# encryptorion-lab/phantom-fhe

Measured on AMD Instinct MI355X. Metric: forward NTT limb-transforms/s at N=2^16, 45 RNS moduli, higher is better.
Workload: dtype u64; 1 GPU; CKKS N=2^16, 45 data limbs (+15 special), forward NTT of a batch of 16 ciphertext polynomials per step (720 limb-transforms, 360 MiB, HBM-resident; configs[2] parameter set); N=65536, limbs=45, special_limbs=15, parallelism=ciphertext-batch x1, launch=K steps enqueued by one library call (2 K eager kernel launches)

## Files before the change

### phantom-fhe_amd/csrc/pha_modup_conv.h

```cpp
#pragma once

namespace pha {

struct ConvLimbRec {
    u64 p, oninv;
    double fq, fqinv;
    uint32_t jo, prime, fpok, pad;
    u64 ratio1;
};
constexpr int kMcsMaxOut = 64;
__device__ __forceinline__ uint32_t uni32(uint32_t x) { return (uint32_t)__builtin_amdgcn_readfirstlane((int)x); }
__device__ __forceinline__ u64 uni64(u64 x) { return ((u64)uni32((uint32_t)(x >> 32)) << 32) | uni32((uint32_t)x); }

constexpr int kMcsWaves = 2;
constexpr int kMcsRegLimbs = 8;
constexpr int kRescRegLimbs = 15;
constexpr int kDownRegLimbs = 8;
constexpr int mcs_reg_limbs(int form) { return form == 1 ? kRescRegLimbs : form == 2 ? kDownRegLimbs : kMcsRegLimbs; }
constexpr int kMcsLogTile = 10;
template <class C, int ISZ_PAD, int FORM = 0>
__global__ __launch_bounds__(C::THREADS) __attribute__((amdgpu_waves_per_eu(kMcsWaves, kMcsWaves)))
void modup_conv_s1_kernel(const NttKArgs k, const ModupConvArgs m) {
    constexpr bool RESC = FORM == 1;
    static_assert(C::STRIDED && C::EPT == 4 && C::NR == 3 && C::r(0) == 2, "radix-4 strided pass, four coefficients per thread");
    constexpr int K = 4, LOGD = C::LOGT - 2;
    using Prog = PassProgram<C, true, EPI_NONE, false, 1, false>;
    extern __shared__ __attribute__((aligned(16))) unsigned char smem[];
    u64 *lds = reinterpret_cast<u64 *>(smem);
    uint2 *s_rows = reinterpret_cast<uint2 *>(smem + (size_t)C::LDS_WORDS * sizeof(u64));
    ConvLimbRec *s_rec = reinterpret_cast<ConvLimbRec *>(s_rows + m.max_osz * kBcRowPad);
    const int tid = threadIdx.x;
    const uint32_t z = blockIdx.z, tile = blockIdx.x;
    const uint32_t ci = z % m.beta, grp = z / m.beta;
    const BConvDev &d = m.convs[ci];
    const uint32_t n = 1u << k.log_n, isz = d.isz, osz = d.osz, pitch = d.row_pad;
    const bool r90 = uni32(d.r90) != 0;
    for (uint32_t e = tid; e < osz * kBcRowPad; e += C::THREADS) {
        const uint32_t j = e / kBcRowPad, i = e % kBcRowPad;
        s_rows[e] = i < pitch ? reinterpret_cast<const uint2 *>(d.mat30)[j * pitch + i] : uint2{0u, 0u};
    }
    for (uint32_t j = tid; j < osz; j += C::THREADS) {
        ConvLimbRec r;
        r.jo = j + (j >= d.pad_start ? d.pad_len : 0);
        r.prime = r.jo >= k.sel.remap_from ? r.jo + k.sel.remap_add : r.jo;
        r.p = k.mod[r.prime].value;
        r.oninv = d.oninv[j];
        r.fpok = 0; r.fq = 0.0; r.fqinv = 0.0; r.pad = 0;
        r.ratio1 = k.mod[r.prime].ratio1;
        if (k.fpinfo) {
            const FpInfo fi = k.fpinfo[r.prime];
            r.fpok = fi.ok; r.fq = fi.q; r.fqinv = fi.qinv;
        }
        s_rec[j] = r;
    }
    int v, hi, lo;
    decode_group<C, 0>(tid, v, hi, lo);
    uint32_t off[K];
#pragma unroll
    for (int kk = 0; kk < K; kk++) off[kk] = (uint32_t)(lo + (kk << LOGD)) * k.t2 + tile * C::V + (uint32_t)v;
    const u64 *src = m.src + (size_t)grp * m.src_group_stride + (size_t)d.src_limb * n;
    u64 *dig = k.out + (size_t)z * k.poly_stride;
    constexpr int RL = mcs_reg_limbs(FORM) < ISZ_PAD ? mcs_reg_limbs(FORM) : ISZ_PAD;
    uint2 *s_in = reinterpret_cast<uint2 *>(s_rec + m.max_osz);
    u32 ylo[RL][K], yhi[RL][K];
#pragma unroll
    for (int i = 0; i < ISZ_PAD; i++)
#pragma unroll
        for (int kk = 0; kk < K; kk++) {
            const u64 y = i < (int)isz ? src[(size_t)i * n + off[kk]] : 0;
            if (i < RL) {
                ylo[i][kk] = (u32)y & 0x3fffffffu;
                yhi[i][kk] = (u32)(y >> 30);
            } else {
                s_in[((i - RL) * K + kk) * C::THREADS + tid] = uint2{(u32)y & 0x3fffffffu, (u32)(y >> 30)};
            }
        }
    if (d.copy_own && m.own) {
        const u64 *own = m.own + (size_t)grp * m.own_group_stride + (size_t)d.src_limb * n;
        for (uint32_t i = 0; i < isz; i++)
#pragma unroll
            for (int kk = 0; kk < K; kk++) dig[(size_t)(d.src_limb + i) * n + off[kk]] = own[(size_t)i * n + off[kk]];
    }
    __syncthreads();
    auto convert4 = [&](uint32_t e, u64 p, u64 oninv, u64 *out) __attribute__((always_inline)) {
        const uint2 *row = s_rows + e * kBcRowPad;
        u64 ll[K], lh[K], hl[K], hh[K];
#pragma unroll
        for (int kk = 0; kk < K; kk++) ll[kk] = lh[kk] = hl[kk] = hh[kk] = 0;
#pragma unroll
// ... 141 lines not shown
```

### phantom-fhe_amd/csrc/pha_modup_ip.h

```cpp
#pragma once

namespace pha {

template <class C, int BETA, bool FP>
__device__ __forceinline__ void modup_ip_body(const NttKArgs &k, const ModupIpArgs &ip, uint32_t twr, uint32_t prime, uint32_t tile,
                                              u64 *lds, int tid) {
    constexpr int RL = C::NR - 1, r = C::r(RL), K = 1 << r, G = C::EPT >> r;
    static_assert(C::LOGT - C::s0(RL) - r == 0, "the last round holds runs of K consecutive coefficients");
    using Prog = PassProgram<C, true, EPI_NONE, false, 0, false>;
    const size_t n = (size_t)1 << k.log_n;
    const DModulus m = k.mod[prime];
    const u64 q = m.value;
    FpMod fm{};
    u64 accb[C::EPT], acca[C::EPT];
#pragma unroll
    for (int i = 0; i < C::EPT; i++) accb[i] = acca[i] = FP ? as_u64(0.0) : 0;
    size_t g0[G];
#pragma unroll
    for (int gi = 0; gi < G; gi++) {
        int v, hi, lo;
        decode_group<C, RL>(tid + C::THREADS * gi, v, hi, lo);
        g0[gi] = ((size_t)tile * C::V + v) * C::T + ((size_t)hi << r);
    }
#pragma unroll 1
    for (int b = 0; b < BETA; b++) {
        PassArgs a;
        full_tile_args<C, true, EPI_NONE, false>(k, twr, (uint32_t)b, tile, a);
        a.fp = FP;
        fm = a.fpm;
        u64 reg[C::EPT];
        if (ip.own && limb_excluded(k, twr, (uint32_t)b)) {
#pragma unroll
            for (int gi = 0; gi < G; gi++)
#pragma unroll
                for (int kk = 0; kk < K; kk += 2) {
                    const u64x2 w = *reinterpret_cast<const u64x2 *>(ip.own + (size_t)twr * n + g0[gi] + kk);
                    reg[gi * K + kk] = FP ? as_u64(fp_from_canon(w.x)) : w.x;
                    reg[gi * K + kk + 1] = FP ? as_u64(fp_from_canon(w.y)) : w.y;
                }
        } else {
            u64x2 twreg[C::TW_TOTAL];
            Prog::load_twiddles(a, tid, twreg);
            Prog::template run_pass<SEG_KEEP, true>(a, lds, tid, reg, twreg);
            if (!FP) {
#pragma unroll
                for (int i = 0; i < C::EPT; i++) reg[i] = csub(csub(csub(reg[i], q << 2), q << 1), q);
            }
        }
        const u64 *key = ip.evks[b];
#pragma unroll
        for (int gi = 0; gi < G; gi++)
#pragma unroll
            for (int kk = 0; kk < K; kk += 2) {
                const size_t id = (size_t)prime * n + g0[gi] + kk;
// ... 113 lines not shown
```

### phantom-fhe_amd/csrc/pha_ntt.hip

```cpp
#include "../../include/phantom_amd.h"
#include "pha_internal.h"
#include "pha_experiments.h"
#include "pha_ntt_core.h"

#include <atomic>
#include <type_traits>

namespace pha {

constexpr int kPassHoist = 0;
#ifndef PHA_NTT_PASS_ORDER
#define PHA_NTT_PASS_ORDER 1
#endif
#ifndef PHA_NTT_ORDER_INT_HEAD
#define PHA_NTT_ORDER_INT_HEAD 1
#endif
#if defined(PHA_EXPERIMENTS)
std::atomic<int> g_ntt_variant{kDefaultVariant};
static inline int ntt_variant() { return g_ntt_variant.load(std::memory_order_relaxed); }
std::atomic<int> g_whole14_min{1 << 30};
std::atomic<int> g_fused_split{0};
std::atomic<int> g_fused_lag{2};
std::atomic<int> g_fused_min_tiles{1 << 30};
extern std::atomic<int> g_bconv_split;
#else
static constexpr int ntt_variant() { return kDefaultVariant; }
#endif

struct NttKArgs {
    const u64 *in;
    u64 *out;
    u64 *mid;
    const u64x2 *tw;
    const DModulus *mod;
    const u64x2 *ninv;
    const u64x2 *w1ninv;
    const u64 *twf;
    const u64x2 *ninvf, *w1ninvf;
    const FpInfo *fpinfo;
    const u64 *scale;
    const u64 *scale_shoup;
    const u64 *aux;
    const u64 *aux2;
// ... 101 lines not shown
        if (EPI == EPI_FWD_KSRESCALE) a.aux2 += (size_t)z * k.aux2_stride;
    }
    if (EPI == EPI_INV_CANON_ADD) a.aux += (size_t)(z >> 1) * k.aux_pair_stride + (size_t)(z & 1) * k.aux_stride;
    if (muladd_epilogue(EPI)) {
        a.aux += (size_t)z * k.aux_stride;
        a.aux2 += (size_t)z * k.aux2_stride;
        if (a.aux3) a.aux3 += (size_t)z * k.aux3_stride;
    }
    if (FWD && (C::STRIDED || C::WHOLE) && k.pro_src) {
        const uint32_t prime = twr >= k.sel.remap_from ? twr + k.sel.remap_add : twr;
        a.in = k.pro_src + (size_t)z * k.pro_stride;
        a.pro_reduce = true;
        a.pro_ratio1 = k.mod[prime].ratio1;
        a.pro_half = bfv_lift_threshold(k.pro_t);
        a.pro_inc = bfv_lift_increment(a.q, k.pro_t);
        a.pro_k = k.pro_k;
        a.ratio0 = k.mod[prime].ratio0;
        a.ratio1 = a.pro_ratio1;
    }
}

template <class C, bool FWD, int EPI, bool FOLD, int HOIST, bool COH, int ONLY = 0, int PRO = PRO_NONE>
__device__ __forceinline__ void exec_pass(const PassArgs &a, u64 *lds, int tid) {
    u64 reg[C::EPT];
    u64x2 twreg[C::TW_TOTAL];
    using Prog = PassProgram<C, FWD, EPI, FOLD, HOIST, COH, PRO>;
    auto pass = [&](const PassArgs &pa) __attribute__((always_inline)) {
        Prog::load_twiddles(pa, tid, twreg);
        Prog::template run_pass<SEG_PLAIN, false>(pa, lds, tid, reg, twreg);
    };
    PHA_WITH_FP_KNOWN(a, ONLY != 2 && a.fp, pass);
}

template <class C, bool FWD, int EPI, bool FOLD>
__global__ __launch_bounds__(C::THREADS) void ntt_zloop_kernel(const NttKArgs k, const ZloopMap m) {
    static_assert(!C::WHOLE, "the batched form exists for the passes of the two-pass plans");
    extern __shared__ __attribute__((aligned(16))) unsigned char smem[];
    u64 *lds = reinterpret_cast<u64 *>(smem);
    __builtin_amdgcn_s_setprio(3);
    const int tid = threadIdx.x;
    uint32_t b = blockIdx.x;
    PassArgs a;
    if (b < m.int_blocks) {
        const uint32_t tile = b % m.tiles, rest = b / m.tiles, z = rest % k.batch, twr = k.sel.start + m.limb[rest / k.batch];
        if (limb_excluded(k, twr, z)) return;
        full_tile_args<C, FWD, EPI, FOLD>(k, twr, z, tile, a);
        exec_pass<C, FWD, EPI, FOLD, 0, false, 2>(a, lds, tid);
        return;
    }
    b -= m.int_blocks;
    const uint32_t tile = b % m.tiles, rest = b / m.tiles, zgroups = (k.batch + m.zper - 1) / m.zper;
    const uint32_t twr = k.sel.start + m.limb[m.n_int + rest / zgroups];
    const uint32_t z0 = (rest % zgroups) * m.zper, z1 = (z0 + m.zper < k.batch) ? z0 + m.zper : k.batch;
    full_tile_args<C, FWD, EPI, FOLD>(k, twr, z0, tile, a);
    using Prog = PassProgram<C, FWD, EPI, FOLD, 1, false>;
    a.fp = true;
    u64x2 twreg[C::TW_TOTAL];
    Prog::load_twiddles(a, tid, twreg);
    u64 regA[C::EPT], regB[C::EPT];
    auto args_of = [&](uint32_t z) __attribute__((always_inline)) {
        PassArgs b = a;
        const size_t dz = (size_t)(z - z0);
        b.in += dz * k.in_stride;
        b.out += dz * k.out_stride;
        if (EPI == EPI_FWD_MODDOWN || EPI == EPI_FWD_MODDOWN_ADD || EPI == EPI_FWD_KSRESCALE) b.aux += dz * k.aux_stride;
        if (EPI == EPI_FWD_KSRESCALE) b.aux2 += dz * k.aux2_stride;
        return b;
    };
    auto transform = [&](const PassArgs &b, u64 *reg) __attribute__((always_inline)) {
        Prog::template run_pass<SEG_PREFETCHED, true>(b, lds, tid, reg, twreg);
    };
    auto next = [&](uint32_t z) __attribute__((always_inline)) {
        while (z < z1 && limb_excluded(k, twr, z)) z++;
        return z;
    };
    uint32_t z = next(z0);
    if (z >= z1) return;
    Prog::prefetch(args_of(z), tid, regA);
    __builtin_amdgcn_s_setprio(0);
    for (;;) {
        uint32_t zn = next(z + 1);
        if (zn < z1) Prog::prefetch(args_of(zn), tid, regB);
        transform(args_of(z), regA);
        if (zn >= z1) break;
        z = zn;
        zn = next(z + 1);
        if (zn < z1) Prog::prefetch(args_of(zn), tid, regA);
        transform(args_of(z), regB);
        if (zn >= z1) break;
        z = zn;
    }
}

template <class C, bool FWD, int EPI, bool FOLD, int HOIST, int PRO = PRO_NONE>
__global__ __launch_bounds__(C::THREADS) void ntt_pass_kernel(const NttKArgs k, const PassOrder o) {
    extern __shared__ __attribute__((aligned(16))) unsigned char smem[];
    u64 *lds = reinterpret_cast<u64 *>(smem);

    __builtin_amdgcn_s_setprio(3);
    uint32_t tile = blockIdx.x, y = blockIdx.y, z = blockIdx.z;
    if (k.zfast_tiles) {
        const uint32_t b = blockIdx.x, per_chunk = k.zfast_run * k.batch, chunk = b / per_chunk, rem = b - chunk * per_chunk;
        z = rem / k.zfast_run;
        const uint32_t group = chunk * k.zfast_run + (rem - z * k.zfast_run);
        if (group >= k.zfast_tiles * k.sel.count) return;
        tile = group % k.zfast_tiles;
        y = group / k.zfast_tiles;
    }
#if PHA_NTT_PASS_ORDER
    else if (o.tiles) {
        if (!pass_order_decode(o, k.batch, blockIdx.x, blockIdx.y, blockIdx.z, y, z, tile)) return;
    }
#endif
    const uint32_t twr = k.sel.start + y;
    if (limb_excluded(k, twr, z)) return;
    PassArgs a;
    full_tile_args<C, FWD, EPI, FOLD>(k, twr, z, tile, a);
    exec_pass<C, FWD, EPI, FOLD, HOIST, false, 0, PRO>(a, lds, threadIdx.x);
}

static void raise_lds_limit(const void *kernel, size_t bytes, std::atomic<uint64_t> &raised) {
// ... 75 lines not shown
    if constexpr (FWD) {
        if (k.pro_small) {
            if constexpr (W::LOGT <= 13) {
                if (epi == EPI_FWD_MULADD) return launch_pass<W, true, EPI_FWD_MULADD, false, PRO_SMALL>(k, s);
                if (epi == EPI_FWD_NEG_MULADD) return launch_pass<W, true, EPI_FWD_NEG_MULADD, false, PRO_SMALL>(k, s);
                return launch_pass<W, true, EPI_FWD_CANON, false, PRO_SMALL>(k, s);
            } else {
                throw std::logic_error("ntt_forward: the sample lift has no one-workgroup form at this degree");
            }
        }
        dispatch_epi<true>(epi, [&](auto e) {
            if constexpr (e() == EPI_FWD_CANON) dispatch_pro(k, [&](auto p) { launch_pass<W, true, EPI_FWD_CANON, false, p()>(k, s); });
            else launch_pass<W, true, e(), false>(k, s);
        });
    } else {
        launch_inverse_last<W>(k, epi, s);
    }
}

template <class C>
static bool plan_zloop(const NttKArgs &k, ZloopMap &m) {
    if (k.pro_src || k.sel.count > 128) return false;
    uint8_t fp[128];
    for (uint32_t y = 0; y < k.sel.count; y++) {
        const uint32_t twr = k.sel.start + y, prime = twr >= k.sel.remap_from ? twr + k.sel.remap_add : twr;
        fp[y] = k.fpinfo != nullptr && (k.h_primes[prime] >> 50) == 0;
    }
    return zloop_plan(m, k.sel.count, fp, k.batch, (uint32_t)(((size_t)1 << k.log_n) >> C::LOGTILE), C::THREADS / 64, kZloopMinBatch);
}
template <class C, bool FWD, int EPI, bool FOLD>
static void launch_zloop(const NttKArgs &k, const ZloopMap &m, hipStream_t s) {
    NttKArgs kk = k;
    kk.zfast_tiles = 0;
    const size_t lds_bytes = (size_t)C::LDS_WORDS * sizeof(u64);
    hipLaunchKernelGGL((ntt_zloop_kernel<C, FWD, EPI, FOLD>), dim3(zloop_blocks(m, k.batch)), dim3(C::THREADS), lds_bytes, s, kk, m);
    check_launch();
}
template <class C>
static void launch_zloop_forward(const NttKArgs &k, const ZloopMap &m, int epi, hipStream_t s) {
    dispatch_epi<true>(epi, [&](auto e) { launch_zloop<C, true, e(), false>(k, m, s); });
}

constexpr size_t kLastLevelCacheBytes = (size_t)256 << 20;
static NttKArgs limb_range(const NttKArgs &k, uint32_t lo, uint32_t cnt) {
    NttKArgs h = k;
    h.sel.start = k.sel.start + lo;
    h.sel.count = cnt;
    return h;
}
static uint32_t order_parts(const NttKArgs &k) {
    const size_t bytes = ((size_t)k.sel.count * k.batch << k.log_n) * sizeof(u64);
    return PHA_NTT_PASS_ORDER == 2 && k.sel.count >= 2 && bytes > kLastLevelCacheBytes ? 2u : 1u;
}

template <class F>
static void for_each_order_part(const NttKArgs &k, const ZloopMap &m, int strided_logtile, F &&pair) {
    if (PHA_NTT_PASS_ORDER == 0) return pair(0u, k.sel.count, m, (const PassOrder *)nullptr);
    const uint32_t parts = order_parts(k), cut = pass_order_half(k.sel.count);
    for (uint32_t h = 0; h < parts; h++) {
        const uint32_t lo = h * cut, hi = parts == 1 ? k.sel.count : h ? k.sel.count : cut;
        const ZloopMap mh = parts == 1 ? m : zloop_sub(m, lo, hi, k.batch);
        const PassOrder o = pass_order_reverse(mh, (uint32_t)(((size_t)1 << k.log_n) >> strided_logtile), PHA_NTT_ORDER_INT_HEAD != 0);
        pair(lo, hi - lo, mh, &o);
    }
}

constexpr int kIpPlan = 3;
// ... 480 lines not shown
```

### phantom-fhe_amd/csrc/pha_ntt_core.h

```cpp
#pragma once
#include "pha_arith.h"
#include "pha_bfv_lift.h"
#include "pha_ckks_fft.h"
#include "pha_encrypt.h"

namespace pha {

constexpr int kTileElems = 4096;

enum Epilogue {
    EPI_NONE = 0,
    EPI_FWD_CANON = 1,
    EPI_FWD_MODDOWN = 2,
    EPI_INV_CANON = 3,
    EPI_INV_SCALE = 4,
    EPI_FWD_MODDOWN_ADD = 5,
    EPI_FWD_KSRESCALE = 6,
    EPI_INV_CANON_ADD = 7,
    EPI_FWD_MULADD = 8,
    EPI_FWD_NEG_MULADD = 9,
};
constexpr bool muladd_epilogue(int epi) { return epi == EPI_FWD_MULADD || epi == EPI_FWD_NEG_MULADD; }

enum Prologue {
    PRO_NONE = 0,
    PRO_LIFT = 1,
    PRO_CKKS = 2,
    PRO_SMALL = 3,
};

template <int LOGT_, bool STRIDED_, int R0_, int R1_, int R2_ = 0, int EPT_ = 16, bool OT_ = false, int LOGTILE_ = 12,
          bool WHOLE_ = false, int R3_ = 0>
struct PassCfg {
    static constexpr int EPT = EPT_;
    static constexpr bool OT = OT_ && !STRIDED_;
    static constexpr int LOGTILE = LOGTILE_;
    static constexpr int TILE = 1 << LOGTILE_;
    static constexpr int THREADS = TILE / EPT_;
    static_assert(LOGTILE_ >= LOGT_ && LOGTILE_ <= 14, "a tile holds whole transforms and fits the LDS budget (2^14 words + padding = 144 KiB of the 160 KiB)");
    static constexpr bool WAVE_LOCAL = TILE / EPT_ == 64;
    static constexpr bool WHOLE = WHOLE_ && !STRIDED_;
    static_assert((1 << R0_) <= EPT_ && (1 << R1_) <= EPT_ && (1 << R2_) <= EPT_ && (1 << R3_) <= EPT_, "radix exceeds registers");
    static_assert(!R3_ || R2_, "rounds are filled in order");
    static constexpr int LOGT = LOGT_;
    static constexpr int T = 1 << LOGT_;
    static constexpr int LOGV = LOGTILE_ - LOGT_;
    static constexpr int V = 1 << LOGV;
    static constexpr bool STRIDED = STRIDED_;
    static constexpr int NR = R3_ ? 4 : R2_ ? 3 : 2;
    static_assert(R0_ + R1_ + R2_ + R3_ == LOGT_, "round schedule must cover all stages");
    static_assert(LOGT_ >= 4 && LOGT_ <= 14, "tile transform length out of range");
    static_assert(THREADS >= 64, "a workgroup is at least one wavefront");
    static constexpr int r(int i) { return i == 0 ? R0_ : i == 1 ? R1_ : i == 2 ? R2_ : R3_; }
    static constexpr bool ot_round(int i) { return OT && i == NR - 1; }
    static constexpr int tw_count(int i) {
        return !r(i) ? 0 : ot_round(i) ? ((1 << r(i)) - 1) + (EPT_ >> r(i)) * r(i) : (EPT_ >> r(i)) * ((1 << r(i)) - 1);
    }
    static constexpr int tw_off(int i) {
        return i == 0 ? 0 : i == 1 ? tw_count(0) : i == 2 ? tw_count(0) + tw_count(1) : tw_count(0) + tw_count(1) + tw_count(2);
    }
    static constexpr int TW_TOTAL = tw_count(0) + tw_count(1) + tw_count(2) + tw_count(3);
    static constexpr int s0(int i) { return i == 0 ? 0 : i == 1 ? R0_ : i == 2 ? R0_ + R1_ : R0_ + R1_ + R2_; }
    static constexpr int PITCH = T + ((T >> 4) << 1);
    static constexpr int LDS_WORDS = STRIDED_ ? (T * V + (T >> 4) * 16) : (V * PITCH);
    static constexpr int lds_index(int e, int v) {
        return STRIDED_ ? (e * V + v + ((e >> 4) << 4)) : (v * PITCH + e + ((e >> 4) << 1));
    }
};

struct PassArgs {
    const u64 *in;
    u64 *out;
    const u64x2 *tw;
    const u64 *twd;
    u64 q;
    u32 tile;
    u32 rho0;
    u32 stride;
    u64x2 ninv, w1ninv;
    u64x2 scale;
    const u64 *aux;
    u64x2 scale2;
    const u64 *aux2;
    bool fp;
    FpMod fpm;
    bool pro_reduce;
    u64 pro_ratio1;
    u64 pro_half, pro_inc;
    u64 pro_k;
    u64 ratio0, ratio1;
    const u64 *aux3;
};

template <class C>
PHA_HD size_t global_index(const PassArgs &a, int e, int v) {
    if (C::STRIDED) return (size_t)e * a.stride + (size_t)a.tile * C::V + v;
    return ((size_t)a.tile * C::V + v) * C::T + e;
}

template <class C, int RI>
PHA_HD void decode_group(int g, int &v, int &hi, int &lo) {
// ... 256 lines not shown
        return u64x2{t.x, t.y};
    }
#endif
    return *p;
}
template <bool NT>
PHA_HD void gstore(u64 *p, u64 v) {
#if defined(__HIP_DEVICE_COMPILE__)
    if (NT) {
        __builtin_nontemporal_store(v, p);
        return;
    }
#endif
    *p = v;
}
template <bool NT>
PHA_HD void gstore2(u64x2 *p, u64x2 v) {
#if defined(__HIP_DEVICE_COMPILE__)
    if (NT) {
        __builtin_nontemporal_store(u64v2{v.x, v.y}, reinterpret_cast<u64v2 *>(p));
        return;
    }
#endif
    *p = v;
}

template <class C, int RI, bool FROM_GLOBAL, bool COH = false>
PHA_HD void round_load(const PassArgs &a, const u64 *lds, int tid, u64 *reg) {
    constexpr int r = C::r(RI), K = 1 << r, G = C::EPT >> r, s0 = C::s0(RI);
    constexpr int LOGD = C::LOGT - s0 - r;
#pragma unroll
    for (int gi = 0; gi < G; gi++) {
        int v, hi, lo;
        decode_group<C, RI>(tid + C::THREADS * gi, v, hi, lo);
        u64 *rg = reg + gi * K;
        const int e0 = (hi << (LOGD + r)) + lo;
        if (FROM_GLOBAL && COH) {
#if defined(__HIP_DEVICE_COMPILE__)
            if constexpr (!C::STRIDED && K == 8 && G == 1 && LOGD >= 1 && LOGD <= 6) {
                const bool odd = lo & 1;
                const u64 *base = a.in + global_index<C>(a, e0 - (odd ? 1 : 0) + ((odd ? 4 : 0) << LOGD), v);
                u64x2 w0, w1, w2, w3;
                asm volatile("global_load_dwordx4 %0, %4, off sc1\n\t"
                             "global_load_dwordx4 %1, %4, off offset:%5 sc1\n\t"
                             "global_load_dwordx4 %2, %4, off offset:%6 sc1\n\t"
                             "global_load_dwordx4 %3, %4, off offset:%7 sc1\n\t"
                             "s_waitcnt vmcnt(0)"
                             : "=&v"(w0), "=&v"(w1), "=&v"(w2), "=&v"(w3)
                             : "v"(base), "n"(8 << LOGD), "n"(16 << LOGD), "n"(24 << LOGD)
                             : "memory");
                const u64x2 w[4] = {w0, w1, w2, w3};
#pragma unroll
                for (int j = 0; j < 4; j++) {
                    const u64 send = odd ? w[j].x : w[j].y;
                    const u32 slo = (u32)__builtin_amdgcn_update_dpp(0, (int)(u32)send, 0xB1, 0xF, 0xF, false);
                    const u32 shi = (u32)__builtin_amdgcn_update_dpp(0, (int)(u32)(send >> 32), 0xB1, 0xF, 0xF, false);
                    const u64 recv = ((u64)shi << 32) | slo;
                    rg[j] = odd ? recv : w[j].x;
                    rg[4 + j] = odd ? w[j].y : recv;
                }
                continue;
            }
#endif
#pragma unroll
            for (int k = 0; k < K; k++) rg[k] = coherent_load(a.in + global_index<C>(a, e0 + (k << LOGD), v));
        } else if (FROM_GLOBAL) {
            if (!C::STRIDED && LOGD == 0) {
                const u64x2 *p = reinterpret_cast<const u64x2 *>(a.in + global_index<C>(a, e0, v));
#pragma unroll
                for (int k = 0; k < K; k += 2) {
                    u64x2 t = gload2<false>(p + (k >> 1));
                    rg[k] = t.x;
                    rg[k + 1] = t.y;
                }
            } else {
#pragma unroll
                for (int k = 0; k < K; k++) rg[k] = gload<false>(a.in + global_index<C>(a, e0 + (k << LOGD), v));
            }
        } else {
#pragma unroll
            for (int k = 0; k < K; k++) rg[k] = lds[C::lds_index(e0 + (k << LOGD), v)];
        }
    }
}

template <class C, int RI>
PHA_HD void round_load_tw(const PassArgs &a, int tid, u64x2 *twreg) {
    constexpr int r = C::r(RI), K = 1 << r, G = C::EPT >> r, s0 = C::s0(RI);
    if (C::ot_round(RI)) {
        static_assert(!C::ot_round(RI) || (C::THREADS % (1 << s0)) == 0, "groups of a thread must share hi");
        u64x2 *base = twreg + C::tw_off(RI);
        int v, hi, lo;
        decode_group<C, RI>(tid, v, hi, lo);
        load_group_twiddles<r>(base, a, (u32)hi);
#pragma unroll
        for (int gi = 0; gi < G; gi++) {
            decode_group<C, RI>(tid + C::THREADS * gi, v, hi, lo);
            const u32 rho = a.rho0 + a.tile * C::V + (u32)v;
#pragma unroll
            for (int j = 0; j < r; j++) base[(K - 1) + gi * r + j] = tw_entry(a, rho << (s0 + j));
        }
        return;
    }
#pragma unroll
    for (int gi = 0; gi < G; gi++) {
        int v, hi, lo;
        decode_group<C, RI>(tid + C::THREADS * gi, v, hi, lo);
        const u32 rho = C::STRIDED ? 1u : (a.rho0 + a.tile * C::V + (u32)v);
        const u32 base0 = (rho << s0) + (u32)hi;
        load_group_twiddles<r>(twreg + C::tw_off(RI) + gi * (K - 1), a, base0);
    }
}

template <class C, int RI, bool FWD, bool FOLD, bool RECENTRE = false, bool GSFULL = false>
PHA_HD void round_compute(const PassArgs &a, int tid, u64 *reg, const u64x2 *twreg) {
    constexpr int r = C::r(RI), K = 1 << r, G = C::EPT >> r;
    const u64 q4 = a.q << 2, nq = 0 - a.q;
    if (C::ot_round(RI)) {
        const u64x2 *tc = twreg + C::tw_off(RI);
#pragma unroll
        for (int gi = 0; gi < G; gi++) {
            u64 *rg = reg + gi * K;
            const u64x2 *tr = tc + (K - 1) + gi * r;
            if (a.fp) {
                if (FWD ? a.fpm.ct_light : a.fpm.gs_light) ot_round_fp<r, FWD, true>(rg, tc, tr, a.fpm);
                else ot_round_fp<r, FWD, false>(rg, tc, tr, a.fpm);
            } else {
                ot_round_int<r, FWD>(rg, tc, tr, q4, nq);
            }
        }
        return;
    }
    if (a.fp) {
#pragma unroll
        for (int gi = 0; gi < G; gi++) {
            u64 *rg = reg + gi * K;
            const u64x2 *t = twreg + C::tw_off(RI) + gi * (K - 1);
            if (FWD) {
                fp_ct_round<r>(rg, t, a.fpm);
                if (RECENTRE && !a.fpm.ct_light) {
// ... 7 lines not shown
                if (light) fp_gs_round<r, FOLD, true>(rg, t, a.fpm, a.ninv, a.w1ninv);
                else fp_gs_round<r, FOLD, false, stage0, canon_in>(rg, t, a.fpm, a.ninv, a.w1ninv);
            } else {
                if (GSFULL) {
                    constexpr bool canon = RI == C::NR - 1 && (!C::STRIDED || C::WHOLE);
                    fp_gs_round<r, FOLD, false, 0, canon>(rg, t, a.fpm, a.ninv, a.w1ninv);
                } else {
                    fp_gs_round<r, FOLD, true>(rg, t, a.fpm, a.ninv, a.w1ninv);
                }
                if (RECENTRE) {
#pragma unroll
                    for (int k = 0; k < K; k++) rg[k] = as_u64(fp_reduce(as_f64(rg[k]), a.fpm));
                }
            }
        }
        return;
    }
#pragma unroll
    for (int gi = 0; gi < G; gi++) {
        u64 *rg = reg + gi * K;
        const u64x2 *t = twreg + C::tw_off(RI) + gi * (K - 1);
        if (FWD) ct_round<r>(rg, t, q4, nq);
        else gs_round<r, FOLD>(rg, t, q4, nq, a.ninv, a.w1ninv);
    }
}

template <class C, int RI, bool TO_GLOBAL, int EPI>
PHA_HD void round_out(const PassArgs &a, u64 *lds, int tid, const u64 *reg) {
    constexpr int r = C::r(RI), K = 1 << r, G = C::EPT >> r, s0 = C::s0(RI);
    constexpr int LOGD = C::LOGT - s0 - r;
#pragma unroll
    for (int gi = 0; gi < G; gi++) {
        int v, hi, lo;
        decode_group<C, RI>(tid + C::THREADS * gi, v, hi, lo);
        const u64 *rg = reg + gi * K;
        const int e0 = (hi << (LOGD + r)) + lo;
        if (TO_GLOBAL) {
            if (!C::STRIDED && LOGD == 0) {
                const size_t g0 = global_index<C>(a, e0, v);
                u64x2 *p = reinterpret_cast<u64x2 *>(a.out + g0);
#pragma unroll
                for (int k = 0; k < K; k += 2) {
                    if constexpr (muladd_epilogue(EPI)) {
                        const bool has_p = EPI == EPI_FWD_NEG_MULADD && a.aux3 != nullptr;
                        const u64x2 f0 = reinterpret_cast<const u64x2 *>(a.aux + g0)[k >> 1], f1 = reinterpret_cast<const u64x2 *>(a.aux2 + g0)[k >> 1];
                        const u64x2 pl = has_p ? reinterpret_cast<const u64x2 *>(a.aux3 + g0)[k >> 1] : u64x2{0, 0};
                        u64x2 t;
                        t.x = apply_epilogue_muladd<EPI>(rg[k], a, f0.x, f1.x, pl.x);
                        t.y = apply_epilogue_muladd<EPI>(rg[k + 1], a, f0.y, f1.y, pl.y);
                        gstore2<false>(p + (k >> 1), t);
                        continue;
                    }
                    u64x2 aux{0, 0}, acc{0, 0};
                    if (EPI == EPI_FWD_MODDOWN || EPI == EPI_FWD_MODDOWN_ADD || EPI == EPI_FWD_KSRESCALE || EPI == EPI_INV_CANON_ADD)
                        aux = reinterpret_cast<const u64x2 *>(a.aux + g0)[k >> 1];
                    if (EPI == EPI_FWD_MODDOWN_ADD) acc = p[k >> 1];
                    if (EPI == EPI_FWD_KSRESCALE) acc = reinterpret_cast<const u64x2 *>(a.aux2 + g0)[k >> 1];
                    u64x2 t;
                    t.x = apply_epilogue_v<EPI>(rg[k], a, aux.x, acc.x);
                    t.y = apply_epilogue_v<EPI>(rg[k + 1], a, aux.y, acc.y);
                    gstore2<false>(p + (k >> 1), t);
                }
            } else {
#pragma unroll
                for (int k = 0; k < K; k++) {
                    const size_t gidx = global_index<C>(a, e0 + (k << LOGD), v);
                    gstore<false>(a.out + gidx, apply_epilogue<EPI>(rg[k], a, gidx));
                }
            }
        } else {
#pragma unroll
            for (int k = 0; k < K; k++) lds[C::lds_index(e0 + (k << LOGD), v)] = rg[k];
        }
    }
}

template <class C>
PHA_HD void tile_sync() {
#if defined(__HIP_DEVICE_COMPILE__)
    if constexpr (C::WAVE_LOCAL) {
        __builtin_amdgcn_fence(__ATOMIC_RELEASE, "wavefront");
        __builtin_amdgcn_wave_barrier();
        __builtin_amdgcn_fence(__ATOMIC_ACQUIRE, "wavefront");
    } else {
        __syncthreads();
    }
#endif
}

enum SegMode { SEG_PLAIN = 0, SEG_PREFETCHED = 1, SEG_KEEP = 2 };

template <class C, bool FWD, int EPI, bool FOLD, int HOIST = 1, bool COH = false, int PRO = PRO_NONE>
struct PassProgram {
    static constexpr int NSEG = C::NR;
    static constexpr int THREADS = C::THREADS;
    static constexpr bool FIRST_PASS = C::WHOLE || (FWD ? C::STRIDED : !C::STRIDED);
    static constexpr bool LAST_PASS = C::WHOLE || !(FWD ? C::STRIDED : !C::STRIDED);

    static constexpr double kFpLimit = 7.5;
    struct FpSched {
        bool recentre[4];
        bool full[4];
        double after[4];
    };
    static constexpr double fp_grow(double m, int stages, bool full) {
        if (!FWD) {
            if (full) return 2.0;
            for (int i = 0; i < stages; i++) m = 2.0 * m + 1e-6;
            return m;
        }
        for (int i = 0; i < stages; i++) m = full ? m + 0.5 + 1e-6 : 1.375 * m + 0.5 + 1e-6;
        return m;
    }
// ... 24 lines not shown
            if (C::ot_round(ri) && (sc.full[seg] || (FWD && sc.recentre[seg]))) return false;
        }
        return true;
    }
    static_assert(fp_sched_ok(), "FP64 path: a round would take the registers past 7.5 q (exactness needs < 8 q at 50 bits), or the schedule asks an on-the-fly-twiddle round to re-centre");

    PHA_HD static void fp_after_global_load(const PassArgs &a, u64 *reg) {
        if (!a.fp) return;
        if (!FIRST_PASS && !(FWD ? a.fpm.ct_light : a.fpm.gs_light)) return;
#pragma unroll
        for (int i = 0; i < C::EPT; i++)
            reg[i] = as_u64(FIRST_PASS ? fp_from_canon(reg[i]) : fp_reduce(as_f64(reg[i]), a.fpm));
    }
    PHA_HD static void fp_before_global_store(const PassArgs &a, u64 *reg) {
        if (!a.fp || !LAST_PASS) return;
        if (fp_epilogue(EPI)) return;
#pragma unroll
        for (int i = 0; i < C::EPT; i++) reg[i] = fp_to_canon(as_f64(reg[i]), a.fpm);
    }

    static constexpr int round_of(int seg) { return FWD ? seg : C::NR - 1 - seg; }
    PHA_HD static void load_twiddles(const PassArgs &a, int tid, u64x2 *twreg) {
        if (HOIST == 1) {
            round_load_tw<C, 0>(a, tid, twreg);
            round_load_tw<C, 1>(a, tid, twreg);
            if (C::NR >= 3) round_load_tw<C, 2>(a, tid, twreg);
            if (C::NR == 4) round_load_tw<C, 3>(a, tid, twreg);
        } else if (HOIST == 2) {
            round_load_tw<C, round_of(0)>(a, tid, twreg);
        }
    }
    template <int SEG>
    PHA_HD static void segment_twiddles(const PassArgs &a, int tid, u64x2 *twreg) {
        if (HOIST == 0) round_load_tw<C, round_of(SEG)>(a, tid, twreg);
        if (HOIST == 2 && SEG + 1 < C::NR) round_load_tw<C, round_of(SEG + 1 < C::NR ? SEG + 1 : SEG)>(a, tid, twreg);
    }

    template <int SEG, int MODE>
    PHA_HD static void segment(const PassArgs &a, u64 *lds, int tid, u64 *reg, u64x2 *twreg) {
        constexpr int RI = round_of(SEG);
        constexpr bool first = SEG == 0, last = SEG == C::NR - 1;
        static_assert(MODE != SEG_KEEP || (last && !first), "the kept segment is the last one of a multi-round pass");
        static_assert(MODE != SEG_KEEP || !(fp_sched().recentre[SEG] || fp_sched().full[SEG]), "a kept segment hands over what the rounds left");
        segment_twiddles<SEG>(a, tid, twreg);
        if constexpr (!(first && MODE == SEG_PREFETCHED)) round_load<C, RI, first, COH>(a, lds, tid, reg);
        if constexpr (first && MODE == SEG_PLAIN) {
#if defined(__HIP_DEVICE_COMPILE__)
            __builtin_amdgcn_s_setprio(0);
#endif
            if constexpr (PRO == PRO_LIFT) {
                static_assert(FWD && FIRST_PASS, "the plain lift is the load prologue of a forward transform's first pass");
#pragma unroll
                for (int i = 0; i < C::EPT; i++) reg[i] = bfv_lift_word(reg[i], a.pro_half, a.pro_inc);
            } else if constexpr (PRO == PRO_CKKS) {
                static_assert(FWD && FIRST_PASS, "round-and-reduce is the load prologue of a forward transform's first pass");
#pragma unroll
                for (int i = 0; i < C::EPT; i++) reg[i] = ckks_round_reduce64(as_f64(reg[i]), a.q, a.pro_ratio1);
            } else if constexpr (PRO == PRO_SMALL) {
                static_assert(FWD && FIRST_PASS, "the sample lift is the load prologue of a forward transform's first pass");
                if (a.pro_k) {
                    const DModulus dm{a.q, a.ratio0, a.ratio1};
                    const u64 kq = barrett64(a.pro_k, a.q, a.ratio1);
#pragma unroll
                    for (int i = 0; i < C::EPT; i++) reg[i] = small_lift_scaled(reg[i], kq, dm);
                } else {
#pragma unroll
                    for (int i = 0; i < C::EPT; i++) reg[i] = small_lift(reg[i], a.q);
                }
            } else if (FWD && FIRST_PASS && a.pro_reduce) {
#pragma unroll
                for (int i = 0; i < C::EPT; i++) reg[i] = barrett64(reg[i], a.q, a.pro_ratio1);
            }
        }
        static_assert(PRO == PRO_NONE || MODE == SEG_PLAIN, "the load prologue belongs to the pass that loads");
        if (first) fp_after_global_load(a, reg);
        if (FWD && C::WHOLE && C::LOGT >= 14 && SEG == 2 && a.fp) {
#pragma unroll
            for (int i = 0; i < C::EPT; i++) reg[i] = as_u64(fp_reduce(as_f64(reg[i]), a.fpm));
        }
        round_compute<C, RI, FWD, FOLD && RI == 0, fp_sched().recentre[SEG], fp_sched().full[SEG]>(a, tid, reg, twreg);
        if constexpr (MODE != SEG_KEEP) {
            if (last) fp_before_global_store(a, reg);
            round_out<C, RI, last, last ? EPI : (int)EPI_NONE>(a, lds, tid, reg);
        }
    }
    template <int SEG>
    PHA_HD static void run(const PassArgs &a, u64 *lds, int tid, u64 *reg, u64x2 *twreg) { segment<SEG, SEG_PLAIN>(a, lds, tid, reg, twreg); }
    template <int SEG>
    PHA_HD static void run_prefetched(const PassArgs &a, u64 *lds, int tid, u64 *reg, u64x2 *twreg) { segment<SEG, SEG_PREFETCHED>(a, lds, tid, reg, twreg); }
    template <int SEG>
    PHA_HD static void run_keep(const PassArgs &a, u64 *lds, int tid, u64 *reg, u64x2 *twreg) { segment<SEG, SEG_KEEP>(a, lds, tid, reg, twreg); }

    PHA_HD static void prefetch(const PassArgs &a, int tid, u64 *reg) { round_load<C, round_of(0), true>(a, nullptr, tid, reg); }

    template <int MODE, bool TAIL_SYNC, int SEG = 0>
    PHA_HD static void run_pass(const PassArgs &a, u64 *lds, int tid, u64 *reg, u64x2 *twreg) {
        constexpr bool last = SEG == NSEG - 1;
        segment<SEG, (MODE == SEG_KEEP && !last) ? (int)SEG_PLAIN : MODE>(a, lds, tid, reg, twreg);
        if constexpr (!last) {
            tile_sync<C>();
            run_pass<MODE, TAIL_SYNC, SEG + 1>(a, lds, tid, reg, twreg);
        } else if constexpr (TAIL_SYNC) {
            tile_sync<C>();
        }
    }
};

#define PHA_WITH_FP_KNOWN(a, cond, body) \
    if (cond) {                          \
        PassArgs b_ = (a);               \
        b_.fp = true;                    \
        body(b_);                        \
    } else {                             \
        PassArgs b_ = (a);               \
        b_.fp = false;                   \
        body(b_);                        \
    }

template <int LOGN, int VARIANT> struct NttPlan;
template <> struct NttPlan<12, 0> { using P1 = PassCfg<6, true, 3, 3>;  using P2 = PassCfg<6, false, 3, 3>; };
template <> struct NttPlan<13, 0> { using P1 = PassCfg<6, true, 3, 3>;  using P2 = PassCfg<7, false, 4, 3>; };
template <> struct NttPlan<14, 0> { using P1 = PassCfg<7, true, 4, 3>;  using P2 = PassCfg<7, false, 4, 3>; };
template <> struct NttPlan<15, 0> { using P1 = PassCfg<7, true, 4, 3>;  using P2 = PassCfg<8, false, 4, 4>; };
template <> struct NttPlan<16, 0> { using P1 = PassCfg<8, true, 4, 4>;  using P2 = PassCfg<8, false, 4, 4>; };
template <> struct NttPlan<17, 0> { using P1 = PassCfg<8, true, 4, 4>;  using P2 = PassCfg<9, false, 3, 3, 3>; };
template <> struct NttPlan<12, 1> { using P1 = PassCfg<6, true, 3, 3, 0, 8>;  using P2 = PassCfg<6, false, 3, 3, 0, 8>; };
template <> struct NttPlan<13, 1> { using P1 = PassCfg<6, true, 3, 3, 0, 8>;  using P2 = PassCfg<7, false, 3, 2, 2, 8>; };
template <> struct NttPlan<14, 1> { using P1 = PassCfg<7, true, 3, 2, 2, 8>;  using P2 = PassCfg<7, false, 3, 2, 2, 8>; };
template <> struct NttPlan<15, 1> { using P1 = PassCfg<7, true, 3, 2, 2, 8>;  using P2 = PassCfg<8, false, 3, 3, 2, 8>; };
template <> struct NttPlan<16, 1> { using P1 = PassCfg<8, true, 3, 3, 2, 8>;  using P2 = PassCfg<8, false, 3, 3, 2, 8>; };
template <> struct NttPlan<17, 1> { using P1 = PassCfg<8, true, 3, 3, 2, 8>;  using P2 = PassCfg<9, false, 3, 3, 3, 8>; };
template <> struct NttPlan<12, 2> { using P1 = PassCfg<6, true, 3, 3, 0, 8>;  using P2 = PassCfg<6, false, 3, 3, 0, 8, true>; };
template <> struct NttPlan<13, 2> { using P1 = PassCfg<6, true, 3, 3, 0, 8>;  using P2 = PassCfg<7, false, 3, 2, 2, 8, true>; };
// ... 169 lines not shown
```

Measured before the change: 2.657 million NTT/s.

## Use wave-local barriers for wave-owned NTT rounds and double-buffer zloop LDS

Remaps thread-to-group assignment so that, in non-strided multi-wave tiles, each wavefront owns contiguous blocks of groups. Later rounds whose data stays inside one wavefront can then synchronise with a wavefront barrier instead of the workgroup barrier. The batched zloop kernel alternates between two LDS areas so the trailing tail barrier can be dropped. A new hoist mode (3) loads the next round's twiddles after compute but is not enabled by default. The doubled LDS footprint could limit occupancy, and a static_assert caps it.

```diff
diff --git a/phantom-fhe_amd/csrc/pha_modup_conv.h b/phantom-fhe_amd/csrc/pha_modup_conv.h
--- a/phantom-fhe_amd/csrc/pha_modup_conv.h
+++ b/phantom-fhe_amd/csrc/pha_modup_conv.h
@@ -54,7 +54,7 @@
         s_rec[j] = r;
     }
     int v, hi, lo;
-    decode_group<C, 0>(tid, v, hi, lo);
+    decode_group<C, 0>(thread_group<C>(tid, 0, 1), v, hi, lo);
     uint32_t off[K];
 #pragma unroll
     for (int kk = 0; kk < K; kk++) off[kk] = (uint32_t)(lo + (kk << LOGD)) * k.t2 + tile * C::V + (uint32_t)v;
diff --git a/phantom-fhe_amd/csrc/pha_modup_ip.h b/phantom-fhe_amd/csrc/pha_modup_ip.h
--- a/phantom-fhe_amd/csrc/pha_modup_ip.h
+++ b/phantom-fhe_amd/csrc/pha_modup_ip.h
@@ -19,7 +19,7 @@
 #pragma unroll
     for (int gi = 0; gi < G; gi++) {
         int v, hi, lo;
-        decode_group<C, RL>(tid + C::THREADS * gi, v, hi, lo);
+        decode_group<C, RL>(thread_group<C>(tid, gi, G), v, hi, lo);
         g0[gi] = ((size_t)tile * C::V + v) * C::T + ((size_t)hi << r);
     }
 #pragma unroll 1
diff --git a/phantom-fhe_amd/csrc/pha_ntt.hip b/phantom-fhe_amd/csrc/pha_ntt.hip
--- a/phantom-fhe_amd/csrc/pha_ntt.hip
+++ b/phantom-fhe_amd/csrc/pha_ntt.hip
@@ -8,7 +8,10 @@
 
 namespace pha {
 
-constexpr int kPassHoist = 0;
+#ifndef PHA_NTT_PASS_HOIST
+#define PHA_NTT_PASS_HOIST 0
+#endif
+constexpr int kPassHoist = PHA_NTT_PASS_HOIST;
 #ifndef PHA_NTT_PASS_ORDER
 #define PHA_NTT_PASS_ORDER 1
 #endif
@@ -176,6 +179,8 @@
     PHA_WITH_FP_KNOWN(a, ONLY != 2 && a.fp, pass);
 }
 
+template <class C>
+constexpr int zloop_areas() { return C::WAVE_LOCAL ? 1 : 2; }
 template <class C, bool FWD, int EPI, bool FOLD>
 __global__ __launch_bounds__(C::THREADS) void ntt_zloop_kernel(const NttKArgs k, const ZloopMap m) {
     static_assert(!C::WHOLE, "the batched form exists for the passes of the two-pass plans");
@@ -189,7 +194,7 @@
         const uint32_t tile = b % m.tiles, rest = b / m.tiles, z = rest % k.batch, twr = k.sel.start + m.limb[rest / k.batch];
         if (limb_excluded(k, twr, z)) return;
         full_tile_args<C, FWD, EPI, FOLD>(k, twr, z, tile, a);
-        exec_pass<C, FWD, EPI, FOLD, 0, false, 2>(a, lds, tid);
+        exec_pass<C, FWD, EPI, FOLD, kPassHoist, false, 2>(a, lds, tid);
         return;
     }
     b -= m.int_blocks;
@@ -211,8 +216,9 @@
         if (EPI == EPI_FWD_KSRESCALE) b.aux2 += dz * k.aux2_stride;
         return b;
     };
-    auto transform = [&](const PassArgs &b, u64 *reg) __attribute__((always_inline)) {
-        Prog::template run_pass<SEG_PREFETCHED, true>(b, lds, tid, reg, twreg);
+    auto transform = [&](const PassArgs &b, u64 *reg, int area) __attribute__((always_inline)) {
+        constexpr bool two = zloop_areas<C>() == 2;
+        Prog::template run_pass<SEG_PREFETCHED, !two>(b, two ? lds + area * C::LDS_WORDS : lds, tid, reg, twreg);
     };
     auto next = [&](uint32_t z) __attribute__((always_inline)) {
         while (z < z1 && limb_excluded(k, twr, z)) z++;
@@ -225,12 +231,12 @@
     for (;;) {
         uint32_t zn = next(z + 1);
         if (zn < z1) Prog::prefetch(args_of(zn), tid, regB);
-        transform(args_of(z), regA);
+        transform(args_of(z), regA, 0);
         if (zn >= z1) break;
         z = zn;
         zn = next(z + 1);
         if (zn < z1) Prog::prefetch(args_of(zn), tid, regA);
-        transform(args_of(z), regB);
+        transform(args_of(z), regB, 1);
         if (zn >= z1) break;
         z = zn;
     }
@@ -372,7 +378,8 @@
 static void launch_zloop(const NttKArgs &k, const ZloopMap &m, hipStream_t s) {
     NttKArgs kk = k;
     kk.zfast_tiles = 0;
-    const size_t lds_bytes = (size_t)C::LDS_WORDS * sizeof(u64);
+    const size_t lds_bytes = (size_t)zloop_areas<C>() * C::LDS_WORDS * sizeof(u64);
+    static_assert(zloop_areas<C>() * C::LDS_WORDS * sizeof(u64) <= 20 * 1024, "eight workgroups per CU (four wavefronts per SIMD of two-wavefront workgroups) need <= 20 KiB each");
     hipLaunchKernelGGL((ntt_zloop_kernel<C, FWD, EPI, FOLD>), dim3(zloop_blocks(m, k.batch)), dim3(C::THREADS), lds_bytes, s, kk, m);
     check_launch();
 }
diff --git a/phantom-fhe_amd/csrc/pha_ntt_core.h b/phantom-fhe_amd/csrc/pha_ntt_core.h
--- a/phantom-fhe_amd/csrc/pha_ntt_core.h
+++ b/phantom-fhe_amd/csrc/pha_ntt_core.h
@@ -40,6 +40,7 @@
     static_assert(LOGTILE_ >= LOGT_ && LOGTILE_ <= 14, "a tile holds whole transforms and fits the LDS budget (2^14 words + padding = 144 KiB of the 160 KiB)");
     static constexpr bool WAVE_LOCAL = TILE / EPT_ == 64;
     static constexpr bool WHOLE = WHOLE_ && !STRIDED_;
+    static constexpr bool WAVE_BLOCKS = !STRIDED_ && !WHOLE_ && LOGTILE_ == LOGT_ && TILE / EPT_ > 64;
     static_assert((1 << R0_) <= EPT_ && (1 << R1_) <= EPT_ && (1 << R2_) <= EPT_ && (1 << R3_) <= EPT_, "radix exceeds registers");
     static_assert(!R3_ || R2_, "rounds are filled in order");
     static constexpr int LOGT = LOGT_;
@@ -61,12 +62,21 @@
     }
     static constexpr int TW_TOTAL = tw_count(0) + tw_count(1) + tw_count(2) + tw_count(3);
     static constexpr int s0(int i) { return i == 0 ? 0 : i == 1 ? R0_ : i == 2 ? R0_ + R1_ : R0_ + R1_ + R2_; }
+    static constexpr int ilog2(int x) { return x <= 1 ? 0 : 1 + ilog2(x >> 1); }
+    static constexpr bool round_is_wave_owned(int i) { return WAVE_LOCAL || (WAVE_BLOCKS && s0(i) >= LOGT_ - ilog2(64 * EPT_)); }
     static constexpr int PITCH = T + ((T >> 4) << 1);
     static constexpr int LDS_WORDS = STRIDED_ ? (T * V + (T >> 4) * 16) : (V * PITCH);
     static constexpr int lds_index(int e, int v) {
         return STRIDED_ ? (e * V + v + ((e >> 4) << 4)) : (v * PITCH + e + ((e >> 4) << 1));
     }
 };
+
+template <class C>
+PHA_HD constexpr int thread_group(int tid, int gi, int G) {
+    return C::WAVE_BLOCKS ? ((tid >> 6) * G + gi) * 64 + (tid & 63) : tid + C::THREADS * gi;
+}
+template <class C>
+constexpr bool exchange_is_wave_local(int i) { return C::round_is_wave_owned(i) && C::round_is_wave_owned(i + 1); }
 
 struct PassArgs {
     const u64 *in;
@@ -389,7 +399,7 @@
 #pragma unroll
     for (int gi = 0; gi < G; gi++) {
         int v, hi, lo;
-        decode_group<C, RI>(tid + C::THREADS * gi, v, hi, lo);
+        decode_group<C, RI>(thread_group<C>(tid, gi, G), v, hi, lo);
         u64 *rg = reg + gi * K;
         const int e0 = (hi << (LOGD + r)) + lo;
         if (FROM_GLOBAL && COH) {
@@ -445,14 +455,14 @@
 PHA_HD void round_load_tw(const PassArgs &a, int tid, u64x2 *twreg) {
     constexpr int r = C::r(RI), K = 1 << r, G = C::EPT >> r, s0 = C::s0(RI);
     if (C::ot_round(RI)) {
-        static_assert(!C::ot_round(RI) || (C::THREADS % (1 << s0)) == 0, "groups of a thread must share hi");
+        static_assert(!C::ot_round(RI) || ((C::WAVE_BLOCKS ? 64 : C::THREADS) % (1 << s0)) == 0, "groups of a thread must share hi");
         u64x2 *base = twreg + C::tw_off(RI);
         int v, hi, lo;
-        decode_group<C, RI>(tid, v, hi, lo);
+        decode_group<C, RI>(thread_group<C>(tid, 0, G), v, hi, lo);
         load_group_twiddles<r>(base, a, (u32)hi);
 #pragma unroll
         for (int gi = 0; gi < G; gi++) {
-            decode_group<C, RI>(tid + C::THREADS * gi, v, hi, lo);
+            decode_group<C, RI>(thread_group<C>(tid, gi, G), v, hi, lo);
             const u32 rho = a.rho0 + a.tile * C::V + (u32)v;
 #pragma unroll
             for (int j = 0; j < r; j++) base[(K - 1) + gi * r + j] = tw_entry(a, rho << (s0 + j));
@@ -462,7 +472,7 @@
 #pragma unroll
     for (int gi = 0; gi < G; gi++) {
         int v, hi, lo;
-        decode_group<C, RI>(tid + C::THREADS * gi, v, hi, lo);
+        decode_group<C, RI>(thread_group<C>(tid, gi, G), v, hi, lo);
         const u32 rho = C::STRIDED ? 1u : (a.rho0 + a.tile * C::V + (u32)v);
         const u32 base0 = (rho << s0) + (u32)hi;
         load_group_twiddles<r>(twreg + C::tw_off(RI) + gi * (K - 1), a, base0);
@@ -536,7 +546,7 @@
 #pragma unroll
     for (int gi = 0; gi < G; gi++) {
         int v, hi, lo;
-        decode_group<C, RI>(tid + C::THREADS * gi, v, hi, lo);
+        decode_group<C, RI>(thread_group<C>(tid, gi, G), v, hi, lo);
         const u64 *rg = reg + gi * K;
         const int e0 = (hi << (LOGD + r)) + lo;
         if (TO_GLOBAL) {
@@ -579,10 +589,13 @@
     }
 }
 
-template <class C>
+constexpr int kTailSync = -1;
+template <class C, int X = kTailSync>
 PHA_HD void tile_sync() {
+    static_assert(X >= kTailSync && X < C::NR - 1, "no such exchange");
+    static_assert(C::WAVE_LOCAL || !exchange_is_wave_local<C>(0), "the first round of several wavefronts spans the tile: its exchange needs the workgroup barrier");
 #if defined(__HIP_DEVICE_COMPILE__)
-    if constexpr (C::WAVE_LOCAL) {
+    if constexpr (X == kTailSync ? C::WAVE_LOCAL : exchange_is_wave_local<C>(X)) {
         __builtin_amdgcn_fence(__ATOMIC_RELEASE, "wavefront");
         __builtin_amdgcn_wave_barrier();
         __builtin_amdgcn_fence(__ATOMIC_ACQUIRE, "wavefront");
@@ -673,7 +686,7 @@
     }
     template <int SEG>
     PHA_HD static void segment_twiddles(const PassArgs &a, int tid, u64x2 *twreg) {
-        if (HOIST == 0) round_load_tw<C, round_of(SEG)>(a, tid, twreg);
+        if (HOIST == 0 || (HOIST == 3 && SEG == 0)) round_load_tw<C, round_of(SEG)>(a, tid, twreg);
         if (HOIST == 2 && SEG + 1 < C::NR) round_load_tw<C, round_of(SEG + 1 < C::NR ? SEG + 1 : SEG)>(a, tid, twreg);
     }
 
@@ -720,6 +733,7 @@
             for (int i = 0; i < C::EPT; i++) reg[i] = as_u64(fp_reduce(as_f64(reg[i]), a.fpm));
         }
         round_compute<C, RI, FWD, FOLD && RI == 0, fp_sched().recentre[SEG], fp_sched().full[SEG]>(a, tid, reg, twreg);
+        if constexpr (HOIST == 3 && !last) round_load_tw<C, round_of(last ? SEG : SEG + 1)>(a, tid, twreg);
         if constexpr (MODE != SEG_KEEP) {
             if (last) fp_before_global_store(a, reg);
             round_out<C, RI, last, last ? EPI : (int)EPI_NONE>(a, lds, tid, reg);
@@ -739,7 +753,7 @@
         constexpr bool last = SEG == NSEG - 1;
         segment<SEG, (MODE == SEG_KEEP && !last) ? (int)SEG_PLAIN : MODE>(a, lds, tid, reg, twreg);
         if constexpr (!last) {
-            tile_sync<C>();
+            tile_sync<C, FWD ? SEG : C::NR - 2 - SEG>();
             run_pass<MODE, TAIL_SYNC, SEG + 1>(a, lds, tid, reg, twreg);
         } else if constexpr (TAIL_SYNC) {
             tile_sync<C>();
```

Result: no change. 2.668 million NTT/s (median of 6 runs) (+0.4%).
